# arkworks-rs/pcd

Hardware: AMD Instinct MI355X
Metric: msm_mscalar_mul_per_s (higher is better)
Workload: dtype u32 (11 x 28-bit unsaturated Montgomery limbs, v_mad_u64_u32 with 64-bit column accumulators); 1 GPU; MNT4-298 G1 variable-base MSM, n=1048576 pairs per GPU (2^20 per GPU), proving-key bases and scalars resident in HBM, scalar distribution uniform; curve=MNT4-298, group=G1, log_n=20, window_bits=20, windows=15

## Files before the change

### pcd_amd/csrc/capi_msm.hip

```cpp
#include <mutex>

#include "capi_internal.h"

using namespace pcd;

namespace {
__global__ void __launch_bounds__(256) zero_flagged_kernel(uint32_t* __restrict__ pts, const uint8_t* __restrict__ flags, size_t n_words,
                                                            uint32_t words_per_point) {
  const size_t i = (size_t)blockIdx.x * blockDim.x + threadIdx.x;
  if (i < n_words && flags[i / words_per_point]) pts[i] = 0;
}

int lane_reserve_of(const pcdhip_ctx* ctx) {
  int r = ctx->lane_reserve;
  if (r < 0) { const char* e = getenv("PCDHIP_LANE_RESERVE"); r = e ? atoi(e) : 8; }
  return r < 0 ? 0 : r;
}
hipStream_t masked_lane_of(int device, int cus, int reserve, hipError_t* err) {
  static std::mutex mu;
  static std::map<std::pair<int, int>, hipStream_t> pool;
  std::lock_guard<std::mutex> lock(mu);
  auto it = pool.find({device, reserve});
  if (it != pool.end()) { *err = hipSuccess; return it->second; }
  std::vector<uint32_t> mask((cus + 31) / 32, 0u);
  for (int i = 0; i < cus - reserve; i++) mask[i / 32] |= 1u << (i % 32);
  hipStream_t s = nullptr;
  *err = hipExtStreamCreateWithCUMask(&s, (uint32_t)mask.size(), mask.data());
  if (*err == hipSuccess) pool[{device, reserve}] = s;
  return s;
}
int make_side_streams(pcdhip_ctx* ctx) {
  int least = 0, greatest = 0;
  TRY(hipDeviceGetStreamPriorityRange(&least, &greatest));
  const bool lane_mode = ctx->g16_schedule == 2;
  int cus = 0;
  if (hipDeviceGetAttribute(&cus, hipDeviceAttributeMultiprocessorCount, ctx->device) != hipSuccess || cus <= 0) cus = 256;
  const int normal = (least + greatest) / 2;
  for (int k = 0; k < 6; k++) {
    int prio = lane_mode ? (k < 2 ? greatest : k < 4 ? normal : least) : (k < 2 ? greatest : k == 2 ? normal : least);
    static const char* side_prio = getenv("PCDHIP_SIDE_PRIO");
    if (side_prio && !strcmp(side_prio, "low")) prio = least;
    if (side_prio && !strcmp(side_prio, "mid")) prio = k < 3 ? normal : least;
    TRY(hipStreamCreateWithPriority(&ctx->g16_streams[k], hipStreamNonBlocking, prio));
    TRY(hipEventCreate(&ctx->g16_begin[k]));
    TRY(hipEventCreate(&ctx->g16_end[k]));
  }
  if (lane_mode) {
    int reserve = lane_reserve_of(ctx);
    if (reserve >= cus) reserve = 0;
    if (reserve > 0) {
      hipError_t e = hipSuccess;
      ctx->lane.stream = masked_lane_of(ctx->device, cus, reserve, &e);
      TRY(e);
    } else {
      TRY(hipStreamCreateWithPriority(&ctx->lane_stream, hipStreamNonBlocking, least));
      ctx->lane.stream = ctx->lane_stream;
    }
    ctx->lane.cus = cus - reserve;
  }
  TRY(hipEventCreateWithFlags(&ctx->g16_ready, hipEventDisableTiming));
  return PCDHIP_OK;
}
}

namespace pcd {
hipError_t zero_flagged(hipStream_t st, uint32_t* pts_dev, uint8_t* flags_dev, const uint8_t* flags_host, size_t n, size_t point_bytes) {
  if (!flags_host || !n) return hipSuccess;
  hipError_t e = hipMemcpyAsync(flags_dev, flags_host, n, hipMemcpyHostToDevice, st);
  if (e != hipSuccess) return e;
  const size_t nw = n * (point_bytes / 4);
  hipLaunchKernelGGL(zero_flagged_kernel, dim3((unsigned)((nw + 255) / 256)), dim3(256), 0, st, pts_dev, flags_dev, nw, (uint32_t)(point_bytes / 4));
  return hipGetLastError();
}

void shard_range(size_t n, size_t g, size_t parts, size_t* lo, size_t* hi) {
  const size_t base = n / parts, rem = n % parts;
  *lo = g * base + std::min(g, rem);
  *hi = *lo + base + (g < rem ? 1 : 0);
}
int bases_upload_single(pcdhip_ctx* ctx, int curve_id, int group_id, const uint64_t* xy, const uint8_t* inf, size_t n, pcdhip_bases** out) {
  BIND();
  const GroupEntry& ge = group_entry(curve_id, group_id);
  const size_t abi_b = (size_t)ge.point_abi_words * 4, int_b = (size_t)ge.base_stride_words * 4;
  pcdhip_bases* b = new (std::nothrow) pcdhip_bases();
  if (!b) return PCDHIP_E_OOM;
  b->curve_id = curve_id; b->group_id = group_id; b->n = n; b->dptr = nullptr; b->c = 0; b->groups = 1;
  if (ctx->precompute != 0 && n >= 64) {
    const bool full = ctx->precompute < 0;
    const int c = ctx->msm_c ? ctx->msm_c : std::max(6, msm_pick_window(n, ge.scalar_bits, full ? 1 : 0) + ctx->msm_c_bias);
    const int W = msm_num_windows(ge.scalar_bits, c);
    b->c = c;
    b->groups = full ? W : std::min(W, ctx->precompute);
  }
  hipError_t e = hipErrorOutOfMemory;
  while (true) {
    const size_t want = std::max<size_t>(n, 1) * int_b * b->groups;
    e = (ctx->precompute_budget && want > ctx->precompute_budget && b->groups > 1) ? hipErrorOutOfMemory : hipMalloc(&b->dptr, want);
    if (e == hipSuccess || b->groups == 1) break;
    (void)hipGetLastError();
    b->groups = (b->groups + 1) / 2;
  }
  if (e != hipSuccess) { (void)hipGetLastError(); delete b; return fail(ctx, e); }
  if (b->groups == 1) b->c = 0;
  e = ctx->aux_ws.ensure(AUX_MISC, std::max<size_t>(n, 1) * (abi_b + 1) + 64);
  char* stage = (char*)ctx->aux_ws.buf[AUX_MISC];
  if (e == hipSuccess) e = hipMemcpyAsync(stage, xy, n * abi_b, hipMemcpyHostToDevice, ctx->stream);
  if (e == hipSuccess) e = zero_flagged(ctx->stream, (uint32_t*)stage, (uint8_t*)stage + n * abi_b, inf, n, abi_b);
  if (e == hipSuccess) e = ge.points_in(ctx->stream, (const uint32_t*)stage, (uint32_t)n, b->dptr);
  if (e == hipSuccess && b->groups > 1) {
    const int W = msm_num_windows(ge.scalar_bits, b->c);
    const int Wg = (W + b->groups - 1) / b->groups;
    e = ge.precompute(ctx->stream, b->dptr, (uint32_t)n, b->groups, b->c * Wg);
  }
  if (e == hipSuccess && inf) {
    std::vector<uint32_t> bits((n + 31) / 32 + 1, 0u);
    bool any = false;
    for (size_t i = 0; i < n; i++) if (inf[i]) { bits[i >> 5] |= 1u << (i & 31); any = true; }
    if (any) {
      e = hipMalloc((void**)&b->inf_bits, bits.size() * 4);
      if (e == hipSuccess) e = hipMemcpyAsync(b->inf_bits, bits.data(), bits.size() * 4, hipMemcpyHostToDevice, ctx->stream);
      if (e == hipSuccess) e = hipStreamSynchronize(ctx->stream);
    }
  }
  if (e == hipSuccess) e = hipStreamSynchronize(ctx->stream);
  if (e != hipSuccess) { (void)hipFree(b->dptr); (void)hipFree(b->inf_bits); delete b; return fail(ctx, e); }
  *out = b;
  return PCDHIP_OK;
}

int msm_common(pcdhip_ctx* ctx, const pcdhip_bases* bases, size_t offset, const uint32_t* scalars_dev, size_t n,
               uint64_t* out_xyz, bool out_on_device) {
  const GroupEntry& ge = group_entry(bases->curve_id, bases->group_id);
  const size_t jac_b = (size_t)ge.point_words / 2 * 3 * 4, jac_abi_b = (size_t)ge.point_abi_words / 2 * 3 * 4;
  TRY(ctx->msm_ws.ensure(WS_OUT, jac_b + jac_abi_b + 64));
  uint32_t* out_dev = (uint32_t*)ctx->msm_ws.buf[WS_OUT];
  uint32_t* out_abi = out_dev + jac_b / 4;
  TRY(ge.msm(ctx->msm_ws, ctx->stream, bases->view(offset), scalars_dev, (uint32_t)n, out_dev, ctx->msm_c, ctx->msm_chunk,
             ctx->msm_sort, ctx->msm_profile ? &ctx->msm_tm : nullptr, nullptr, MSM_SHARE_NONE));
  if (out_on_device) { TRY(ge.jac_out(ctx->stream, out_dev, 1, (uint32_t*)out_xyz)); return PCDHIP_OK; }
  TRY(ge.jac_out(ctx->stream, out_dev, 1, out_abi));
  TRY(hipMemcpyAsync(out_xyz, out_abi, jac_abi_b, hipMemcpyDeviceToHost, ctx->stream));
  uint32_t too_wide = 0;
  if (ctx->msm_ws.last_err_dev) TRY(hipMemcpyAsync(&too_wide, ctx->msm_ws.last_err_dev, 4, hipMemcpyDeviceToHost, ctx->stream));
  TRY(hipStreamSynchronize(ctx->stream));
  return too_wide ? PCDHIP_E_ARG : PCDHIP_OK;
}

int ensure_side_streams(pcdhip_ctx* ctx) {
// ... 152 lines not shown
  uint32_t* d = (uint32_t*)ctx->aux_ws.buf[AUX_MISC];
  uint32_t* scratch = d + (n + 1) * jb / 4;
  const uint32_t* in = (const uint32_t*)xyz;
  if (!in_on_device) {
    TRY(hipMemcpyAsync(d + jb / 4, xyz, n * jb, hipMemcpyHostToDevice, ctx->stream));
    in = d + jb / 4;
  }
  TRY(ge.points_sum(ctx->stream, in, (uint32_t)n, scratch, d));
  TRY(hipMemcpyAsync(out_xyz, d, jb, hipMemcpyDeviceToHost, ctx->stream));
  TRY(hipStreamSynchronize(ctx->stream));
  return PCDHIP_OK;
}
}

extern "C" {

int pcdhip_bases_upload(pcdhip_ctx* ctx, int curve_id, int group_id, const uint64_t* xy, const uint8_t* inf, size_t n,
                        pcdhip_bases** out) {
  if (!ctx || !out || !valid_curve(curve_id) || !valid_group(group_id) || (!xy && n) || n >= (1ull << 31)) return PCDHIP_E_ARG;
  if (ctx->peers.size() <= 1) return bases_upload_single(ctx, curve_id, group_id, xy, inf, n, out);
  *out = nullptr;
  return guarded([&]() -> int {
    pcdhip_bases* b = new pcdhip_bases();
    b->curve_id = curve_id; b->group_id = group_id; b->n = n; b->dptr = nullptr; b->c = 0; b->groups = 1;
    const size_t G = ctx->peers.size(), pl = (size_t)pcdhip_point_limbs(curve_id, group_id);
    b->shard_lo.resize(G + 1);
    for (size_t g = 0; g < G; g++) {
      size_t lo, hi;
      shard_range(n, g, G, &lo, &hi);
      b->shard_lo[g] = lo; b->shard_lo[g + 1] = hi;
      pcdhip_ctx* C = ctx->peers[g];
      C->precompute = ctx->precompute; C->precompute_budget = ctx->precompute_budget; C->msm_c = ctx->msm_c;
      pcdhip_bases* sh = nullptr;
      int rc = bases_upload_single(C, curve_id, group_id, xy + lo * pl, inf ? inf + lo : nullptr, hi - lo, &sh);
      if (rc) { pcdhip_bases_free(ctx, b); return rc; }
      b->shards.push_back(sh);
    }
    *out = b;
    return PCDHIP_OK;
  });
}
int pcdhip_set_precompute(pcdhip_ctx* ctx, int mode) {
  if (!ctx || mode < -1 || mode == 1) return PCDHIP_E_ARG;
  ctx->precompute = mode;
  return PCDHIP_OK;
}
int pcdhip_set_precompute_budget(pcdhip_ctx* ctx, size_t bytes_per_vector) {
  if (!ctx) return PCDHIP_E_ARG;
  ctx->precompute_budget = bytes_per_vector;
  return PCDHIP_OK;
}
int pcdhip_get_precompute_budget(pcdhip_ctx* ctx, size_t* bytes_per_vector) {
  if (!ctx || !bytes_per_vector) return PCDHIP_E_ARG;
  *bytes_per_vector = ctx->precompute_budget;
  return PCDHIP_OK;
}
void pcdhip_bases_free(pcdhip_ctx* ctx, pcdhip_bases* bases) {
  if (!bases) return;
  for (size_t g = 0; g < bases->shards.size(); g++)
    pcdhip_bases_free(ctx && g < ctx->peers.size() ? ctx->peers[g] : ctx, bases->shards[g]);
  bases->shards.clear();
  if (ctx) (void)hipSetDevice(ctx->device);
  (void)hipFree(bases->dptr);
  (void)hipFree(bases->inf_bits);
  delete bases;
}
int pcdhip_bases_info(const pcdhip_bases* bases, size_t n, int* window_bits, int* windows, int* copies) {
  if (!bases || !window_bits || !windows || !copies) return PCDHIP_E_ARG;
  if (!bases->shards.empty()) return pcdhip_bases_info(bases->shards[0], 0, window_bits, windows, copies);
  const GroupEntry& ge = group_entry(bases->curve_id, bases->group_id);
  const int c = bases->groups > 1 ? bases->c : msm_pick_window(n ? n : bases->n, ge.scalar_bits, 0);
  *window_bits = c;
  *windows = msm_num_windows(ge.scalar_bits, c);
  *copies = bases->groups;
  return PCDHIP_OK;
}
int pcdhip_msm_config(pcdhip_ctx* ctx, int window_bits, int chunk) {
  if (!ctx || window_bits < 0 || window_bits > 24 || chunk < 0) return PCDHIP_E_ARG;
  ctx->msm_c = window_bits;
  ctx->msm_chunk = (uint32_t)chunk;
  return PCDHIP_OK;
}
int pcdhip_msm_set_sort(pcdhip_ctx* ctx, int mode) {
  if (!ctx || mode < 0 || mode > 2) return PCDHIP_E_ARG;
  ctx->msm_sort = (ctx->msm_sort & ~15) | mode;
  return PCDHIP_OK;
}
int pcdhip_msm_set_accumulate(pcdhip_ctx* ctx, int mode, int chunk, int min_pairs) {
  if (!ctx || mode < 0 || mode > 2 || chunk < 0 || chunk > 1024 || (chunk && chunk < 2) || min_pairs < 0 || min_pairs > 255) return PCDHIP_E_ARG;
  ctx->msm_sort = (ctx->msm_sort & 15) | (mode << 4) | (chunk << 8) | (min_pairs << 20);
  return PCDHIP_OK;
}
int pcdhip_msm_profile(pcdhip_ctx* ctx, int on) {
  if (!ctx) return PCDHIP_E_ARG;
  ctx->msm_profile = on != 0;
  return PCDHIP_OK;
}
int pcdhip_msm_last_plan(pcdhip_ctx* ctx, uint32_t out[2]) {
  if (!ctx || !out) return PCDHIP_E_ARG;
  out[0] = ctx->msm_tm.entries; out[1] = ctx->msm_tm.chunk;
  return PCDHIP_OK;
}
int pcdhip_msm_last_timings(pcdhip_ctx* ctx, float out_ms[8]) {
  if (!ctx || !out_ms) return PCDHIP_E_ARG;
  const MsmTimings& t = ctx->msm_tm;
  float v[8] = {t.digits, t.scan, t.scatter, t.accumulate, t.fixup, t.tail, t.horner, t.total};
  memcpy(out_ms, v, sizeof v);
  return PCDHIP_OK;
}

int pcdhip_msm_ticket_status(pcdhip_ctx* ctx, int slot) {
  if (!ctx || slot < 0 || slot >= pcdhip_ctx::PIPE_SLOTS || ctx->pipe_busy[slot] || !ctx->pipe_partial[slot]) return PCDHIP_E_ARG;
  BIND();
  TRY(hipEventSynchronize(ctx->pipe_done[slot]));
  ctx->pipe_partial[slot] = false;
  return (uint32_t)ctx->pipe_host[(size_t)slot * pcdhip_ctx::PIPE_HOST_WORDS + pcdhip_ctx::PIPE_HOST_WORDS - 1] ? PCDHIP_E_PREV_TICKET : PCDHIP_OK;
}
int pcdhip_msm_submit(pcdhip_ctx* ctx, const pcdhip_bases* bases, size_t offset, const pcdhip_buf* scalars, size_t scalar_offset, size_t n,
                      int* ticket) {
  const int rc = msm_submit_common(ctx, bases, offset, scalars, scalar_offset, n, nullptr, 0, ticket);
  return rc == PCDHIP_E_PREV_TICKET ? PCDHIP_OK : rc;
}
int pcdhip_msm_submit_partial(pcdhip_ctx* ctx, const pcdhip_bases* bases, size_t offset, const pcdhip_buf* scalars, size_t scalar_offset, size_t n,
                              uint64_t* out_xyz_device_slots, size_t slot_stride_bytes, int* ticket) {
  if (!out_xyz_device_slots || (slot_stride_bytes & 7)) return PCDHIP_E_ARG;
  return msm_submit_common(ctx, bases, offset, scalars, scalar_offset, n, out_xyz_device_slots, slot_stride_bytes, ticket);
}
int pcdhip_msm_ticket_wait(pcdhip_ctx* ctx, int ticket, void* other_stream) {
  if (!ctx || ticket < 0 || ticket >= pcdhip_ctx::PIPE_SLOTS || !ctx->pipe_busy[ticket]) return PCDHIP_E_ARG;
  BIND();
  TRY(hipStreamWaitEvent((hipStream_t)other_stream, ctx->pipe_done[ticket], 0));
  ctx->pipe_busy[ticket] = false;
  ctx->pipe_partial[ticket] = true;
  return PCDHIP_OK;
}
int pcdhip_msm_collect(pcdhip_ctx* ctx, int ticket, uint64_t* out_xyz) {
  if (!ctx || ticket < 0 || ticket >= pcdhip_ctx::PIPE_SLOTS || !ctx->pipe_busy[ticket] || !out_xyz) return PCDHIP_E_ARG;
  BIND();
  ctx->pipe_busy[ticket] = false;
  TRY(hipEventSynchronize(ctx->pipe_done[ticket]));
  const uint64_t* host = ctx->pipe_host + (size_t)ticket * pcdhip_ctx::PIPE_HOST_WORDS;
  memcpy(out_xyz, host, ctx->pipe_out_bytes[ticket]);
  return (uint32_t)host[pcdhip_ctx::PIPE_HOST_WORDS - 1] ? PCDHIP_E_ARG : PCDHIP_OK;
}

int pcdhip_msm_dev(pcdhip_ctx* ctx, const pcdhip_bases* bases, size_t offset, const pcdhip_buf* scalars, size_t scalar_offset,
                   size_t n, uint64_t* out_xyz) {
  if (!ctx || !bases || !scalars || !out_xyz) return PCDHIP_E_ARG;
  if (!bases->shards.empty()) return PCDHIP_E_ARG;
  if (offset + n > bases->n || scalar_offset + n > scalars->n || n >= (1ull << 31)) return PCDHIP_E_ARG;
  if (scalars->field_id != kCurveFr[bases->curve_id]) return PCDHIP_E_ARG;
  BIND();
  const size_t sw = (size_t)kFieldLimbs[scalars->field_id] * 2;
  return msm_common(ctx, bases, offset, scalars->dptr + scalar_offset * sw, n, out_xyz);
}

int pcdhip_msm_dev_partial(pcdhip_ctx* ctx, const pcdhip_bases* bases, size_t offset, const pcdhip_buf* scalars, size_t scalar_offset,
                           size_t n, uint64_t* out_xyz_device) {
  if (!ctx || !bases || !scalars || !out_xyz_device || !bases->shards.empty()) return PCDHIP_E_ARG;
  if (offset + n > bases->n || scalar_offset + n > scalars->n || n >= (1ull << 31)) return PCDHIP_E_ARG;
  if (scalars->field_id != kCurveFr[bases->curve_id]) return PCDHIP_E_ARG;
  BIND();
  const size_t sw = (size_t)kFieldLimbs[scalars->field_id] * 2;
  return msm_common(ctx, bases, offset, scalars->dptr + scalar_offset * sw, n, out_xyz_device, true);
}

int pcdhip_msm(pcdhip_ctx* ctx, const pcdhip_bases* bases, size_t offset, const uint64_t* scalars, size_t n, uint64_t* out_xyz) {
// ... 42 lines not shown
```

### pcd_amd/csrc/msm.hip.h

```cpp
#pragma once
#include <cstdlib>
#include <math.h>

#include <algorithm>
#include <type_traits>
#include <vector>

#include "ec.hip.h"

namespace pcd {

template <int K>
struct EventSet {
  hipEvent_t e[K] = {};
  bool live = false;
  hipError_t create() {
    for (int i = 0; i < K; i++) { hipError_t r = hipEventCreate(&e[i]); if (r != hipSuccess) return r; }
    live = true;
    return hipSuccess;
  }
  hipEvent_t operator[](int i) const { return e[i]; }
  ~EventSet() { for (int i = 0; i < K; i++) if (e[i]) (void)hipEventDestroy(e[i]); }
};

struct MsmPlan {
  uint32_t n = 0;
  int c = 0;
  int W = 0;
  uint32_t nkeys = 0;
  uint32_t chunk = 0;
};

PCD_HD constexpr int msm_num_windows(int scalar_bits, int c) { return (scalar_bits + c) / c; }

inline int msm_pick_window(size_t n, int scalar_bits, int full_precompute) {
  double best = 1e300;
  int bc = 8;
  for (int c = 6; c <= 22; c++) {
    int W = msm_num_windows(scalar_bits, c);
    int Wg = full_precompute ? 1 : W;
    double cost = (double)W * (double)n * 11.0 + (double)Wg * (double)(1u << c) * 16.0 * 1.3;
    int top = scalar_bits + 1 - (W - 1) * c;
    cost += (double)n / (double)(1u << (top > 20 ? 20 : top)) * 1400.0;
    if (cost < best) { best = cost; bc = c; }
  }
  return bc;
}

constexpr uint32_t MSM_NEG = 0x80000000u;
PCD_DEV uint32_t msm_signed(uint32_t raw, int c, uint32_t& carry, uint32_t& neg) {
  uint32_t d = raw + carry;
  const bool n = d > (1u << (c - 1));
  carry = n ? 1u : 0u;
  neg = n ? MSM_NEG : 0u;
  return n ? (1u << c) - d : d;
}
template <int NS>
PCD_DEV bool msm_scalar_too_wide(const uint32_t* s, int bits) {
  uint32_t o = 0;
#pragma unroll
  for (int k = 0; k < NS; k++) {
    if (32 * k >= bits) o |= s[k];
    else if (32 * (k + 1) > bits) o |= s[k] >> (bits - 32 * k);
  }
  return o != 0;
}
PCD_DEV bool msm_base_is_inf(const uint32_t* __restrict__ inf_bits, uint32_t idx) { return inf_bits && ((inf_bits[idx >> 5] >> (idx & 31u)) & 1u); }
template <int NS>
PCD_DEV uint32_t msm_digit(const uint32_t* s, int w, int c) {
  int bit = w * c;
  int word = bit >> 5, off = bit & 31;
  uint64_t x = s[word];
  if (word + 1 < NS) x |= (uint64_t)s[word + 1] << 32;
  return (uint32_t)(x >> off) & ((1u << c) - 1u);
}

enum { MODE_HIST = 0, MODE_SCATTER = 1, MODE_BIN = 2 };
template <int NS, int MODE>
__global__ void __launch_bounds__(256) msm_digits_kernel(const uint32_t* __restrict__ scalars, uint32_t n, int c, int W, int Wg,
                                                         uint32_t n_total, uint32_t base_offset, uint32_t nkeys,
                                                         uint32_t* __restrict__ cnt, const uint32_t* __restrict__ off,
                                                         uint32_t* __restrict__ sorted_idx, uint32_t* __restrict__ slots, uint32_t cap,
                                                         uint32_t* __restrict__ ones_idx, uint32_t* __restrict__ flag, int skip_ones,
                                                         int scalar_bits, uint32_t* __restrict__ err, const uint32_t* __restrict__ inf_bits) {
  if (MODE == MODE_SCATTER && flag && *flag == 0) return;
  uint32_t i = blockIdx.x * blockDim.x + threadIdx.x;
  bool live = i < n && !msm_base_is_inf(inf_bits, base_offset + i);
// ... 52 lines not shown
constexpr uint32_t MSM_MAX_BINS = 8192;

template <int NS, bool WRITE>
__global__ void __launch_bounds__(256) msm_coarse_kernel(const uint32_t* __restrict__ scalars, uint32_t n, int c, int W, int Wg,
                                                         uint32_t n_total, uint32_t base_offset, uint32_t nbins,
                                                         uint32_t* __restrict__ gbin ,
                                                         uint64_t* __restrict__ entries, uint32_t* __restrict__ ones_count,
                                                         uint32_t* __restrict__ ones_idx, int scalar_bits, uint32_t* __restrict__ err,
                                                         const uint32_t* __restrict__ inf_bits) {
  extern __shared__ uint32_t lbin[];
  __shared__ uint32_t s_ones[WRITE ? 1 : MSM_TILE];
  __shared__ uint32_t s_nones, s_ones_base;
  for (uint32_t b = threadIdx.x; b < nbins; b += blockDim.x) lbin[b] = 0;
  if (threadIdx.x == 0) s_nones = 0;
  __syncthreads();
  const uint32_t tile0 = blockIdx.x * MSM_TILE;
  for (uint32_t k = threadIdx.x; k < MSM_TILE; k += blockDim.x) {
    uint32_t i = tile0 + k;
    bool live = i < n && !msm_base_is_inf(inf_bits, base_offset + i);
    uint32_t s[NS];
    bool is_one = false;
    if (live || (i < n && !WRITE)) {
      uint32_t hi = 0;
#pragma unroll
      for (int q = 0; q < NS; q++) { s[q] = scalars[(size_t)i * NS + q]; if (q) hi |= s[q]; }
      is_one = live && (hi == 0 && s[0] == 1);
      if (!WRITE && msm_scalar_too_wide<NS>(s, scalar_bits)) *err = 1u;
    }
    if (!WRITE) {
      unsigned long long m = __ballot(live && is_one);
      if (m) {
        int lane = threadIdx.x & 63;
        int leader = __ffsll((long long)m) - 1;
        uint32_t base = 0;
        if (lane == leader) base = atomicAdd(&s_nones, (uint32_t)__popcll(m));
        base = __shfl(base, leader, 64);
        if (live && is_one) s_ones[base + (uint32_t)__popcll(m & ((1ull << lane) - 1ull))] = base_offset + i;
      }
    }
    if (!live || is_one) continue;
    int j = 0;
    uint32_t carry = 0, neg;
    for (int w = 0; w < W; w++) {
      uint32_t d = msm_signed(msm_digit<NS>(s, w, c), c, carry, neg);
      if (d != 0) atomicAdd(&lbin[((((uint32_t)j << c) | d)) >> MSM_BIN_SHIFT], 1u);
      if (++j == Wg) j = 0;
    }
  }
  __syncthreads();
  for (uint32_t b = threadIdx.x; b < nbins; b += blockDim.x) {
    uint32_t cnt = lbin[b];
    if (cnt) {
      uint32_t base = atomicAdd(&gbin[b], cnt);
      if (WRITE) lbin[b] = base;
    }
  }
  if (!WRITE) {
    if (threadIdx.x == 0) s_ones_base = s_nones ? atomicAdd(ones_count, s_nones) : 0u;
    __syncthreads();
    for (uint32_t k = threadIdx.x; k < s_nones; k += blockDim.x) ones_idx[s_ones_base + k] = s_ones[k];
    return;
  }
  __syncthreads();
  for (uint32_t k = threadIdx.x; k < MSM_TILE; k += blockDim.x) {
    uint32_t i = tile0 + k;
    if (i >= n || msm_base_is_inf(inf_bits, base_offset + i)) continue;
    uint32_t s[NS];
    uint32_t hi = 0;
#pragma unroll
    for (int q = 0; q < NS; q++) { s[q] = scalars[(size_t)i * NS + q]; if (q) hi |= s[q]; }
    if (hi == 0 && s[0] <= 1) continue;
    int g = 0, j = 0;
    uint32_t carry = 0, neg;
    for (int w = 0; w < W; w++) {
      uint32_t d = msm_signed(msm_digit<NS>(s, w, c), c, carry, neg);
      if (d != 0) {
        uint32_t key = ((uint32_t)j << c) | d;
        uint32_t pos = atomicAdd(&lbin[key >> MSM_BIN_SHIFT], 1u);
        entries[pos] = ((uint64_t)key << 32) | (uint64_t)(((uint32_t)g * n_total + base_offset + i) | neg);
      }
      if (++j == Wg) { j = 0; g++; }
    }
  }
}

static __global__ void __launch_bounds__(1024) msm_bin_scan_kernel(const uint32_t* __restrict__ bin_cnt, uint32_t nbins,
                                                                   uint32_t* __restrict__ bin_base, uint32_t* __restrict__ cursor,
                                                                   const uint32_t* __restrict__ ones_count, uint32_t* __restrict__ off,
                                                                   uint32_t nkeys) {
  __shared__ uint32_t part[1024];
  const uint32_t per = (nbins + 1023) / 1024;
  const uint32_t lo = threadIdx.x * per, hi = min(nbins, lo + per);
  uint32_t acc = 0;
  for (uint32_t b = lo; b < hi; b++) acc += bin_cnt[b];
  part[threadIdx.x] = acc;
  __syncthreads();
  for (int s = 1; s < 1024; s <<= 1) {
    uint32_t t = ((int)threadIdx.x >= s) ? part[threadIdx.x - s] : 0;
    __syncthreads();
    part[threadIdx.x] += t;
    __syncthreads();
  }
  uint32_t run = part[threadIdx.x] - acc;
  for (uint32_t b = lo; b < hi; b++) { bin_base[b] = run; cursor[b] = run; run += bin_cnt[b]; }
  if (threadIdx.x == 1023) {
    uint32_t M = part[1023];
    bin_base[nbins] = M;
    off[nkeys] = M;
    off[nkeys + 1] = M + *ones_count;
  }
}

static __global__ void __launch_bounds__(256) msm_bin_sort_kernel(const uint64_t* __restrict__ entries, const uint32_t* __restrict__ bin_base,
                                                                  uint32_t* __restrict__ sorted_idx, uint32_t* __restrict__ off) {
  constexpr uint32_t KB = 1u << MSM_BIN_SHIFT;
  __shared__ uint32_t hist[KB];
  __shared__ uint32_t wsum[4];
  const uint32_t b = blockIdx.x, lo = bin_base[b], hi = bin_base[b + 1];
  for (uint32_t k = threadIdx.x; k < KB; k += blockDim.x) hist[k] = 0;
  __syncthreads();
  for (uint32_t p0 = lo + threadIdx.x; p0 < hi; p0 += MSM_SORT_UNROLL * blockDim.x) {
    uint32_t kk[MSM_SORT_UNROLL];
#pragma unroll
    for (int u = 0; u < MSM_SORT_UNROLL; u++) { uint32_t p = p0 + u * blockDim.x; kk[u] = p < hi ? (uint32_t)(entries[p] >> 32) & (KB - 1) : KB; }
#pragma unroll
    for (int u = 0; u < MSM_SORT_UNROLL; u++) if (kk[u] < KB) atomicAdd(&hist[kk[u]], 1u);
  }
  __syncthreads();
  const uint32_t t = threadIdx.x, lane = t & 63, wv = t >> 6;
  uint32_t c0 = hist[2 * t], c1 = hist[2 * t + 1];
  uint32_t incl = c0 + c1;
  for (int d = 1; d < 64; d <<= 1) { uint32_t o = __shfl_up(incl, d, 64); if ((int)lane >= d) incl += o; }
  if (lane == 63) wsum[wv] = incl;
  __syncthreads();
  uint32_t before = 0;
  for (uint32_t q = 0; q < wv; q++) before += wsum[q];
  uint32_t ex = lo + before + incl - (c0 + c1);
  hist[2 * t] = ex;
  hist[2 * t + 1] = ex + c0;
  off[(size_t)b * KB + 2 * t] = ex;
  off[(size_t)b * KB + 2 * t + 1] = ex + c0;
  __syncthreads();
  for (uint32_t p0 = lo + threadIdx.x; p0 < hi; p0 += MSM_SORT_UNROLL * blockDim.x) {
    uint64_t e[MSM_SORT_UNROLL];
    uint32_t pos[MSM_SORT_UNROLL];
#pragma unroll
    for (int u = 0; u < MSM_SORT_UNROLL; u++) { uint32_t p = p0 + u * blockDim.x; e[u] = p < hi ? entries[p] : ~0ull; }
#pragma unroll
    for (int u = 0; u < MSM_SORT_UNROLL; u++) if (e[u] != ~0ull) pos[u] = atomicAdd(&hist[(uint32_t)(e[u] >> 32) & (KB - 1)], 1u);
#pragma unroll
    for (int u = 0; u < MSM_SORT_UNROLL; u++) if (e[u] != ~0ull) sorted_idx[pos[u]] = (uint32_t)e[u];
  }
}

static __global__ void __launch_bounds__(1024) scan_block_sums(const uint32_t* __restrict__ in, uint32_t n, uint32_t per_block,
                                                         uint32_t* __restrict__ block_sums) {
  __shared__ uint32_t sh[1024];
  uint32_t b = blockIdx.x, lo = b * per_block, hi = min(n, lo + per_block);
  uint32_t acc = 0;
  for (uint32_t i = lo + threadIdx.x; i < hi; i += blockDim.x) acc += in[i];
  sh[threadIdx.x] = acc;
  __syncthreads();
  for (int s = 512; s > 0; s >>= 1) { if ((int)threadIdx.x < s) sh[threadIdx.x] += sh[threadIdx.x + s]; __syncthreads(); }
  if (threadIdx.x == 0) block_sums[b] = sh[0];
}
static __global__ void __launch_bounds__(1024) scan_apply(const uint32_t* __restrict__ in, uint32_t n, uint32_t per_block,
// ... 1055 lines not shown
  const bool single_pass = sort_mode == 1;
  const uint32_t* bases_dev = bv.dptr;
  typedef typename G::F F;
  constexpr int NS = G::FR::N32;
  constexpr int PW = Jac<F>::WORDS;
  constexpr size_t PB = (size_t)PW * 4;
  if (n == 0) { ws.last_err_dev = nullptr; Jac<F> inf = Jac<F>::infinity(); return hipMemcpyAsync(out_dev, &inf, PB, hipMemcpyHostToDevice, st); }
  MsmPlan pl;
  pl.n = n;
  pl.c = bv.groups > 1 ? bv.c : (c_override ? c_override : msm_pick_window(n, G::FR::BITS, 0));
  pl.W = msm_num_windows(G::FR::BITS, pl.c);
  const int Wg = (pl.W + bv.groups - 1) / bv.groups;
  pl.nkeys = (uint32_t)Wg << pl.c;
  const uint64_t maxM = (uint64_t)n * pl.W;
  pl.chunk = chunk_override ? chunk_override : 40;
  int& cus = ws.cus;
  if (!cus) {
    int dev = 0;
    if (hipGetDevice(&dev) != hipSuccess || hipDeviceGetAttribute(&cus, hipDeviceAttributeMultiprocessorCount, dev) != hipSuccess || cus <= 0) cus = 256;
  }
  bool use_tree = false;
  uint32_t tree_cap = 0;
  const uint32_t* tree_chunk_dev = nullptr;
  if constexpr (MsmTreeCapable<G>::value) {
    use_tree = acc_mode == 2 && (uint64_t)bv.n_total * bv.groups < MSM_SCR;
    if (use_tree) {
      tree_cap = tree_chunk ? tree_chunk : MSM_TREE_CHUNK_MAX;
      pl.chunk = tree_cap;
    }
  }
  const MsmLane* lane = ws.lane;
  const int plan_cus = lane && lane->cus > 0 ? lane->cus : cus;
  uint32_t acc_lanes = 0, chunk_lo = 0;
  static const uint32_t chunk_hi_env = getenv("PCDHIP_CHUNK_HI") ? (uint32_t)atoi(getenv("PCDHIP_CHUNK_HI")) : 0u;
  const uint32_t chunk_hi = chunk_hi_env >= 16 && chunk_hi_env <= MSM_CHUNK_MAX ? chunk_hi_env : MSM_CHUNK_HI;
  if (!chunk_override && !use_tree) {
    acc_lanes = (uint32_t)plan_cus * 4 * MsmAccWaves<G>::value * (64 / AccOf<G>::LANES);
    chunk_lo = (uint32_t)std::min<uint64_t>(40, std::max<uint64_t>(16, (maxM + 4ull * acc_lanes - 1) / (4ull * acc_lanes)));
    pl.chunk = chunk_lo;
  }
  const uint64_t plan_word = acc_lanes && acc_lanes < (1u << 20) ? msm_plan_word(acc_lanes, chunk_lo, chunk_hi) : 0u;
  if (acc_lanes && !plan_word) pl.chunk = 40;
  if (maxM >= 0xFFFFFFF0ull || (uint64_t)bv.n_total * bv.groups >= 0x7FFFFFF0ull) return hipErrorInvalidValue;

  EventSet<9> ev;
  if (tm) PCD_HIP_TRY(ev.create());
  auto mark = [&](int i) -> hipError_t { return tm ? hipEventRecord(ev[i], st) : hipSuccess; };

  const uint32_t tkeys = pl.nkeys + 1, ones_key = pl.nkeys;
  const bool consume = share && share_role == MSM_SHARE_CONSUME && share->valid && share->n == n && share->n_total == bv.n_total &&
                       share->offset == bv.offset && share->tkeys == tkeys && share->c == pl.c && share->W == pl.W &&
                       share->groups == bv.groups && share->scalars == scalars_dev &&
                       (share->inf_bits == nullptr || share->inf_bits == bv.inf_bits);
  PCD_HIP_TRY(ws.ensure(WS_CNT, (size_t)tkeys * 4 + 16));
  PCD_HIP_TRY(ws.ensure(WS_OFF, ((size_t)tkeys + 1) * 4));
  const uint32_t scan_per_block = 16384;
  const uint32_t scan_blocks = (tkeys + scan_per_block - 1) / scan_per_block;
  PCD_HIP_TRY(ws.ensure(WS_BSUM, (size_t)scan_blocks * 4));
  PCD_HIP_TRY(ws.ensure(WS_SORTED, (size_t)maxM * 4));
  PCD_HIP_TRY(ws.ensure(WS_BUCKETS, (size_t)tkeys * PB));
  PCD_HIP_TRY(ws.ensure(WS_OUT, PB + 64));
  PCD_HIP_TRY(ws.ensure(WS_ONES, (size_t)n * 4 + 32));
  uint32_t* cnt = (uint32_t*)ws.buf[WS_CNT];
  uint32_t* off = (uint32_t*)ws.buf[WS_OFF];
  uint32_t* bsum = (uint32_t*)ws.buf[WS_BSUM];
  uint32_t* sorted = (uint32_t*)ws.buf[WS_SORTED];
  uint32_t* buckets = (uint32_t*)ws.buf[WS_BUCKETS];
  uint32_t* ones_idx = (uint32_t*)ws.buf[WS_ONES];
  uint32_t* flag = ones_idx + n;
  uint32_t* err = flag + 1;
  uint32_t* big_count = flag + 2;
  auto zero_start = [&](uint32_t n_cnt) {
    hipLaunchKernelGGL(msm_zero_kernel, dim3(std::max<uint32_t>(1u, (n_cnt + 255) / 256)), dim3(256), 0, st, cnt, n_cnt, flag);
  };
  ws.last_err_dev = consume ? nullptr : err;
  constexpr int SBITS = G::FR::BITS;
  const int wins = (pl.W + Wg - 1) / Wg;
  const int top_bits = G::FR::BITS + 1 - (pl.W - 1) * pl.c;
  double mu = (double)n * wins / (double)(1u << (pl.c - 1)) + (top_bits < pl.c ? (double)n / (double)(1u << top_bits) : 0.0);
  uint32_t cap = (uint32_t)(mu + 6.0 * sqrt(mu) + 8.0);
  cap = (cap + 7u) & ~7u;
  const bool use_slots = single_pass && (double)pl.nkeys * cap * 4.0 <= 1.5e9;
  const uint32_t nbins = pl.nkeys >> MSM_BIN_SHIFT;
  const bool use_partition = sort_mode == 0 && pl.c >= MSM_BIN_SHIFT && nbins >= 1 && nbins <= MSM_MAX_BINS && n >= 4096;
  uint32_t* slots = nullptr;
  if (use_slots) { PCD_HIP_TRY(ws.ensure(WS_SLOTS, (size_t)pl.nkeys * cap * 4)); slots = (uint32_t*)ws.buf[WS_SLOTS]; }

  PCD_HIP_TRY(mark(0));
  dim3 gd((n + 255) / 256), bd(256);
  MsmEntrySource src;
  if (consume) {
    PCD_HIP_TRY(hipStreamWaitEvent(st, share->ready, 0));
    zero_start(0);
    src = share->src;
    off = const_cast<uint32_t*>(share->off);
    PCD_HIP_TRY(mark(1)); PCD_HIP_TRY(mark(2)); PCD_HIP_TRY(mark(3));
  } else if (use_slots) {
    zero_start(tkeys);
    hipLaunchKernelGGL((msm_digits_kernel<NS, MODE_BIN>), gd, bd, 0, st, scalars_dev, n, pl.c, pl.W, Wg, bv.n_total, bv.offset, pl.nkeys, cnt,
                       (const uint32_t*)nullptr, (uint32_t*)nullptr, slots, cap, ones_idx, flag, 0, SBITS, err, bv.inf_bits);
    PCD_HIP_TRY(mark(1));
    hipLaunchKernelGGL(scan_block_sums, dim3(scan_blocks), dim3(1024), 0, st, cnt, tkeys, scan_per_block, bsum);
    hipLaunchKernelGGL(scan_apply, dim3(scan_blocks), dim3(1024), 0, st, cnt, tkeys, scan_per_block, bsum, scan_blocks, off);
    PCD_HIP_TRY(mark(2));
    PCD_HIP_TRY(ws.ensure(WS_CUR, (size_t)tkeys * 4));
    uint32_t* cur = (uint32_t*)ws.buf[WS_CUR];
    PCD_HIP_TRY(hipMemsetAsync(cur, 0, (size_t)tkeys * 4, st));
    hipLaunchKernelGGL((msm_digits_kernel<NS, MODE_SCATTER>), gd, bd, 0, st, scalars_dev, n, pl.c, pl.W, Wg, bv.n_total, bv.offset, pl.nkeys, cur,
                       off, sorted, (uint32_t*)nullptr, 0u, (uint32_t*)nullptr, flag, 1, SBITS, err, bv.inf_bits);
    PCD_HIP_TRY(mark(3));
    src = {sorted, slots, ones_idx, flag, cap, ones_key};
  } else if (use_partition) {
    zero_start(nbins + 1);
    const uint32_t tiles = (n + MSM_TILE - 1) / MSM_TILE;
    PCD_HIP_TRY(ws.ensure(WS_ENTRIES, (size_t)maxM * 8));
    PCD_HIP_TRY(ws.ensure(WS_CUR, ((size_t)2 * nbins + 8) * 4));
    uint64_t* entries = (uint64_t*)ws.buf[WS_ENTRIES];
    uint32_t* bin_base = (uint32_t*)ws.buf[WS_CUR];
    uint32_t* cursor = bin_base + nbins + 2;
    uint32_t* ones_count = flag;
    hipLaunchKernelGGL((msm_coarse_kernel<NS, false>), dim3(tiles), dim3(256), (size_t)nbins * 4, st, scalars_dev, n, pl.c, pl.W, Wg, bv.n_total,
                       bv.offset, nbins, cnt, (uint64_t*)nullptr, ones_count, ones_idx, SBITS, err, bv.inf_bits);
    PCD_HIP_TRY(mark(1));
    hipLaunchKernelGGL(msm_bin_scan_kernel, dim3(1), dim3(1024), 0, st, cnt, nbins, bin_base, cursor, ones_count, off, pl.nkeys);
    PCD_HIP_TRY(mark(2));
    hipLaunchKernelGGL((msm_coarse_kernel<NS, true>), dim3(tiles), dim3(256), (size_t)nbins * 4, st, scalars_dev, n, pl.c, pl.W, Wg, bv.n_total,
                       bv.offset, nbins, cursor, entries, ones_count, ones_idx, SBITS, err, bv.inf_bits);
    hipLaunchKernelGGL(msm_bin_sort_kernel, dim3(nbins), dim3(256), 0, st, entries, bin_base, sorted, off);
    PCD_HIP_TRY(mark(3));
    src = {sorted, nullptr, ones_idx, nullptr, 0u, ones_key};
  } else {
    zero_start(tkeys);
    hipLaunchKernelGGL((msm_digits_kernel<NS, MODE_HIST>), gd, bd, 0, st, scalars_dev, n, pl.c, pl.W, Wg, bv.n_total, bv.offset, pl.nkeys, cnt,
                       (const uint32_t*)nullptr, (uint32_t*)nullptr, (uint32_t*)nullptr, 0u, (uint32_t*)nullptr, (uint32_t*)nullptr, 0, SBITS, err, bv.inf_bits);
    PCD_HIP_TRY(mark(1));
    hipLaunchKernelGGL(scan_block_sums, dim3(scan_blocks), dim3(1024), 0, st, cnt, tkeys, scan_per_block, bsum);
    hipLaunchKernelGGL(scan_apply, dim3(scan_blocks), dim3(1024), 0, st, cnt, tkeys, scan_per_block, bsum, scan_blocks, off);
    PCD_HIP_TRY(mark(2));
    PCD_HIP_TRY(hipMemsetAsync(cnt, 0, (size_t)tkeys * 4, st));
    hipLaunchKernelGGL((msm_digits_kernel<NS, MODE_SCATTER>), gd, bd, 0, st, scalars_dev, n, pl.c, pl.W, Wg, bv.n_total, bv.offset, pl.nkeys, cnt,
                       off, sorted, (uint32_t*)nullptr, 0u, (uint32_t*)nullptr, (uint32_t*)nullptr, 0, SBITS, err, bv.inf_bits);
    PCD_HIP_TRY(mark(3));
    src = {sorted, nullptr, nullptr, nullptr, 0u, ones_key};
  }
  if (share && share_role == MSM_SHARE_PRODUCE) {
    share->valid = true;
    share->n = n; share->n_total = bv.n_total; share->offset = bv.offset; share->tkeys = tkeys;
    share->c = pl.c; share->W = pl.W; share->groups = bv.groups; share->scalars = scalars_dev; share->inf_bits = bv.inf_bits;
    share->src = src; share->off = off;
    PCD_HIP_TRY(hipEventRecord(share->ready, st));
  }
  uint32_t nchunks = (uint32_t)((maxM + pl.chunk - 1) / pl.chunk);
  uint32_t tree_grid = 0;
  if (use_tree) {
    tree_grid = std::min<uint32_t>(tree_chunk ? (nchunks + 63) / 64 : (uint32_t)((maxM / 32 + 63) / 64), (uint32_t)plan_cus * 4);
    if (!tree_chunk) nchunks = tree_grid * 64 * (uint32_t)((maxM + (uint64_t)tree_grid * 64 * tree_cap - 1) / ((uint64_t)tree_grid * 64 * tree_cap));
  }
  typedef MsmStored<typename SplitOf<G>::type> Stored;
  constexpr size_t RB = (size_t)Stored::WORDS * 4;
  PCD_HIP_TRY(ws.ensure(WS_PFIRST, (size_t)nchunks * RB));
  PCD_HIP_TRY(ws.ensure(WS_PLAST, (size_t)nchunks * RB));
  uint32_t* acc_buckets = buckets;
  if (Stored::SEPARATE) { PCD_HIP_TRY(ws.ensure(WS_ACCB, (size_t)tkeys * RB)); acc_buckets = (uint32_t*)ws.buf[WS_ACCB]; }
  const uint32_t big_limit = 8, seg_len = 128;
  const uint32_t big_cap = nchunks / big_limit + 2;
  const uint32_t seg_cap = nchunks / seg_len + big_cap + 2;
  PCD_HIP_TRY(ws.ensure(WS_BIG, (size_t)(3 * big_cap + 3 * seg_cap + 8) * 4));
  PCD_HIP_TRY(ws.ensure(WS_BIGPART, (size_t)seg_cap * PB));
  uint32_t* pfirst = (uint32_t*)ws.buf[WS_PFIRST];
  uint32_t* plast = (uint32_t*)ws.buf[WS_PLAST];
  uint32_t* big = (uint32_t*)ws.buf[WS_BIG];
  uint32_t* seg_list = big + 3 * big_cap;
  uint32_t* big_partial = (uint32_t*)ws.buf[WS_BIGPART];
  PCD_HIP_TRY(mark(8));
  hipStream_t own = st;
  if (lane) {
    if (!ws.lane_in) PCD_HIP_TRY(hipEventCreateWithFlags(&ws.lane_in, hipEventDisableTiming));
    if (!ws.lane_out) PCD_HIP_TRY(hipEventCreateWithFlags(&ws.lane_out, hipEventDisableTiming));
    PCD_HIP_TRY(hipEventRecord(ws.lane_in, own));
    PCD_HIP_TRY(hipStreamWaitEvent(lane->stream, ws.lane_in, 0));
    st = lane->stream;
  }
  {
    constexpr uint32_t per_wave = 64 / AccOf<G>::LANES;
    const dim3 acc_grid((nchunks + per_wave - 1) / per_wave);
    bool launched = false;
    if constexpr (MsmTreeCapable<G>::value) {
      if (use_tree) {
        constexpr int FW = AccOf<G>::type::F::WORDS;
        const uint32_t grid = tree_grid;
        MsmTreeBufs tb;
        tb.cap = tree_cap;
        tb.phases = 3;
        uint32_t* chunk_word = big_count + 2;
        hipLaunchKernelGGL(msm_tree_plan_kernel, dim3(1), dim3(1), 0, st, off, tkeys, grid * 64, tree_cap, tree_chunk, chunk_word);
        tree_chunk_dev = chunk_word;
        PCD_HIP_TRY(ws.ensure(WS_TLIST, MsmTreeBufs::list_words(tb.cap) * 4 * grid));
        PCD_HIP_TRY(ws.ensure(WS_TPAIR, MsmTreeBufs::pair_words(tb.cap) * 4 * grid));
        PCD_HIP_TRY(ws.ensure(WS_TPREFIX, MsmTreeBufs::prefix_words(tb.cap, FW) * 4 * grid));
        PCD_HIP_TRY(ws.ensure(WS_TPTS, MsmTreeBufs::pts_words(tb.cap, FW) * 4 * grid));
        tb.list = (uint32_t*)ws.buf[WS_TLIST]; tb.pairs = (uint32_t*)ws.buf[WS_TPAIR];
        tb.prefix = (uint32_t*)ws.buf[WS_TPREFIX]; tb.pts = (uint32_t*)ws.buf[WS_TPTS];
        hipLaunchKernelGGL((msm_pair_tree_kernel<G>), dim3(grid), dim3(64), 0, st, bases_dev, src, off, tkeys, chunk_word, tb,
                           tree_min_pairs ? tree_min_pairs : MSM_TREE_MIN_PAIRS, acc_buckets, pfirst, plast);
        launched = true;
      }
    }
    if (!launched) {
      if (src.slots) hipLaunchKernelGGL((msm_accumulate_kernel<G, false>), acc_grid, dim3(64), 0, st, bases_dev, src, off, tkeys, pl.chunk, acc_buckets, pfirst, plast, plan_word);
      hipLaunchKernelGGL((msm_accumulate_kernel<G, true>), acc_grid, dim3(64), 0, st, bases_dev, src, off, tkeys, pl.chunk, acc_buckets, pfirst, plast, plan_word);
// ... 94 lines not shown
```

Baseline: 398.7 Mscalar-mul/s.

## Stage coarse-partition scatter in LDS to write contiguous per-bin runs

Adds a staged coarse scatter kernel for the partition sort path. Each block histograms its tile's digits in LDS and reserves one global range per bin with a single atomic. It then packs entries into an LDS buffer ordered by bin and writes them out as contiguous runs, replacing per-entry global atomics and scattered 64-bit writes. The trade-off is large dynamic LDS use (up to 152 KB), which lowers occupancy, plus a binary search per entry. An env knob can cap or disable the tile, and sort mode 3 keeps the old path.

```diff
diff --git a/pcd_amd/csrc/capi_msm.hip b/pcd_amd/csrc/capi_msm.hip
--- a/pcd_amd/csrc/capi_msm.hip
+++ b/pcd_amd/csrc/capi_msm.hip
@@ -64,6 +64,16 @@
 }
 
 namespace pcd {
+int msm_coarse_tile_knob() {
+  static const int knob = [] {
+    const char* e = getenv("PCDHIP_COARSE_TILE");
+    if (!e || *e < '0' || *e > '9') return -1;
+    const int v = atoi(e);
+    return v == 0 || (v >= (int)MSM_STAGE_TILE_MIN && v <= (int)MSM_STAGE_TILE_MAX) ? v : -1;
+  }();
+  return knob;
+}
+
 hipError_t zero_flagged(hipStream_t st, uint32_t* pts_dev, uint8_t* flags_dev, const uint8_t* flags_host, size_t n, size_t point_bytes) {
   if (!flags_host || !n) return hipSuccess;
   hipError_t e = hipMemcpyAsync(flags_dev, flags_host, n, hipMemcpyHostToDevice, st);
@@ -382,7 +392,7 @@
   return PCDHIP_OK;
 }
 int pcdhip_msm_set_sort(pcdhip_ctx* ctx, int mode) {
-  if (!ctx || mode < 0 || mode > 2) return PCDHIP_E_ARG;
+  if (!ctx || mode < 0 || mode > 3) return PCDHIP_E_ARG;
   ctx->msm_sort = (ctx->msm_sort & ~15) | mode;
   return PCDHIP_OK;
 }
diff --git a/pcd_amd/csrc/msm.hip.h b/pcd_amd/csrc/msm.hip.h
--- a/pcd_amd/csrc/msm.hip.h
+++ b/pcd_amd/csrc/msm.hip.h
@@ -3,6 +3,7 @@
 #include <math.h>
 
 #include <algorithm>
+#include <atomic>
 #include <type_traits>
 #include <vector>
 
@@ -221,6 +222,134 @@
       if (++j == Wg) { j = 0; g++; }
     }
   }
+}
+
+constexpr int MSM_STAGE_G_BITS = 6, MSM_STAGE_IDX_BITS = 11;
+constexpr uint32_t MSM_STAGE_TILE_MAX = 1u << MSM_STAGE_IDX_BITS, MSM_STAGE_TILE_MIN = 256;
+constexpr int MSM_STAGE_W_MAX = 1 << MSM_STAGE_G_BITS;
+constexpr int MSM_STAGE_SIGN_AT = MSM_BIN_SHIFT, MSM_STAGE_G_AT = MSM_BIN_SHIFT + 1, MSM_STAGE_IDX_AT = MSM_STAGE_G_AT + MSM_STAGE_G_BITS;
+static_assert(MSM_STAGE_IDX_AT + MSM_STAGE_IDX_BITS <= 32, "staged word: low key bits, sign, group and tile index in 32 bits");
+constexpr size_t MSM_STAGE_LDS_BUDGET = 152u * 1024u;
+constexpr uint32_t MSM_STAGE_MIN_RUN = 8;
+PCD_HD constexpr size_t msm_stage_lds_bytes(uint32_t tile, int W, uint32_t nbins) { return 4 * ((size_t)tile * (size_t)W + 3 * (size_t)nbins + 4); }
+PCD_HD constexpr uint32_t msm_stage_tile(int W, uint32_t nbins) {
+  if (W < 1 || W > MSM_STAGE_W_MAX || nbins < 1) return 0;
+  for (uint32_t t = MSM_STAGE_TILE_MAX; t >= MSM_STAGE_TILE_MIN; t >>= 1)
+    if (msm_stage_lds_bytes(t, W, nbins) <= MSM_STAGE_LDS_BUDGET) return (uint64_t)t * (uint32_t)W >= (uint64_t)MSM_STAGE_MIN_RUN * nbins ? t : 0;
+  return 0;
+}
+int msm_coarse_tile_knob();
+
+constexpr int msm_stage_block(int TILE) { return TILE < 1024 ? TILE : 1024; }
+template <int NS, int TILE>
+__global__ void __launch_bounds__(msm_stage_block(TILE)) msm_coarse_staged_kernel(const uint32_t* __restrict__ scalars, uint32_t n, int c, int W, int Wg,
+                                                                                  uint32_t n_total, uint32_t base_offset, uint32_t nbins,
+                                                                                  uint32_t* __restrict__ gbin ,
+                                                                                  uint64_t* __restrict__ entries, const uint32_t* __restrict__ inf_bits) {
+  constexpr int BLOCK = msm_stage_block(TILE), K = TILE / BLOCK, NW = BLOCK / 64;
+  static_assert(TILE >= (int)MSM_STAGE_TILE_MIN && TILE <= (int)MSM_STAGE_TILE_MAX && TILE % BLOCK == 0, "tile");
+  extern __shared__ uint32_t lds[];
+  uint32_t* cur = lds;
+  uint32_t* loff = cur + nbins;
+  uint32_t* rdelta = loff + nbins + 1;
+  uint32_t* buf = rdelta + nbins;
+  __shared__ uint32_t s_wsum[NW];
+  const uint32_t t = threadIdx.x, tile0 = blockIdx.x * TILE;
+  for (uint32_t b = t; b < nbins; b += BLOCK) cur[b] = 0;
+  uint32_t s[K][NS];
+  bool live[K];
+#pragma unroll
+  for (int kk = 0; kk < K; kk++) {
+    const uint32_t i = tile0 + t + kk * BLOCK;
+    live[kk] = i < n && !msm_base_is_inf(inf_bits, base_offset + i);
+    uint32_t hi = 0;
+#pragma unroll
+    for (int q = 0; q < NS; q++) { s[kk][q] = live[kk] ? scalars[(size_t)i * NS + q] : 0u; if (q) hi |= s[kk][q]; }
+    if (hi == 0 && s[kk][0] <= 1) live[kk] = false;
+  }
+  __syncthreads();
+#pragma unroll
+  for (int kk = 0; kk < K; kk++) {
+    if (!live[kk]) continue;
+    int j = 0;
+    uint32_t carry = 0, neg;
+    for (int w = 0; w < W; w++) {
+      uint32_t d = msm_signed(msm_digit<NS>(s[kk], w, c), c, carry, neg);
+      if (d != 0) atomicAdd(&cur[((((uint32_t)j << c) | d)) >> MSM_BIN_SHIFT], 1u);
+      if (++j == Wg) j = 0;
+    }
+  }
+  __syncthreads();
+  const uint32_t per = (nbins + BLOCK - 1) / BLOCK;
+  const uint32_t blo = min(nbins, t * per), bhi = min(nbins, blo + per);
+  uint32_t acc = 0;
+  for (uint32_t b = blo; b < bhi; b++) acc += cur[b];
+  const uint32_t lane = t & 63, wv = t >> 6;
+  uint32_t incl = acc;
+  for (int d = 1; d < 64; d <<= 1) { uint32_t o = __shfl_up(incl, d, 64); if ((int)lane >= d) incl += o; }
+  if (lane == 63) s_wsum[wv] = incl;
+  __syncthreads();
+  uint32_t run = incl - acc;
+  for (uint32_t q = 0; q < wv; q++) run += s_wsum[q];
+  for (uint32_t b = blo; b < bhi; b++) {
+    const uint32_t cnt = cur[b];
+    loff[b] = run;
+    cur[b] = run;
+    if (cnt) rdelta[b] = atomicAdd(&gbin[b], cnt) - run;
+    run += cnt;
+  }
+  if (t == BLOCK - 1) loff[nbins] = run;
+  __syncthreads();
+#pragma unroll
+  for (int kk = 0; kk < K; kk++) {
+    if (!live[kk]) continue;
+    int g = 0, j = 0;
+    uint32_t carry = 0, neg;
+    for (int w = 0; w < W; w++) {
+      uint32_t d = msm_signed(msm_digit<NS>(s[kk], w, c), c, carry, neg);
+      if (d != 0) {
+        const uint32_t key = ((uint32_t)j << c) | d;
+        const uint32_t q = atomicAdd(&cur[key >> MSM_BIN_SHIFT], 1u);
+        buf[q] = (key & ((1u << MSM_BIN_SHIFT) - 1u)) | (neg ? 1u << MSM_STAGE_SIGN_AT : 0u) | ((uint32_t)g << MSM_STAGE_G_AT) |
+                 ((t + kk * BLOCK) << MSM_STAGE_IDX_AT);
+      }
+      if (++j == Wg) { j = 0; g++; }
+    }
+  }
+  __syncthreads();
+  const uint32_t total = loff[nbins];
+  for (uint32_t q = t; q < total; q += BLOCK) {
+    const uint32_t word = buf[q];
+    uint32_t lo = 0, hi = nbins;
+    while (hi - lo > 1) {
+      const uint32_t mid = (lo + hi) >> 1;
+      if (loff[mid] <= q) lo = mid; else hi = mid;
+    }
+    const uint32_t key = (lo << MSM_BIN_SHIFT) | (word & ((1u << MSM_BIN_SHIFT) - 1u));
+    const uint32_t g = (word >> MSM_STAGE_G_AT) & ((1u << MSM_STAGE_G_BITS) - 1u);
+    const uint32_t neg = (word >> MSM_STAGE_SIGN_AT) & 1u ? MSM_NEG : 0u;
+    const uint32_t idx = (g * n_total + base_offset + tile0 + (word >> MSM_STAGE_IDX_AT)) | neg;
+    entries[rdelta[lo] + q] = ((uint64_t)key << 32) | (uint64_t)idx;
+  }
+}
+template <int NS, int TILE>
+hipError_t msm_coarse_staged_launch(hipStream_t st, uint32_t tiles, size_t lds, const uint32_t* scalars, uint32_t n, int c, int W, int Wg,
+                                    uint32_t n_total, uint32_t base_offset, uint32_t nbins, uint32_t* gbin, uint64_t* entries,
+                                    const uint32_t* inf_bits) {
+  static std::atomic<uint64_t> allowed{0};
+  int dev = 0;
+  hipError_t e = hipGetDevice(&dev);
+  if (e != hipSuccess) return e;
+  const uint64_t bit = 1ull << (dev & 63);
+  if (!(allowed.load(std::memory_order_relaxed) & bit)) {
+    e = hipFuncSetAttribute(reinterpret_cast<const void*>(&msm_coarse_staged_kernel<NS, TILE>), hipFuncAttributeMaxDynamicSharedMemorySize,
+                            (int)MSM_STAGE_LDS_BUDGET);
+    if (e != hipSuccess) return e;
+    allowed.fetch_or(bit, std::memory_order_relaxed);
+  }
+  hipLaunchKernelGGL((msm_coarse_staged_kernel<NS, TILE>), dim3(tiles), dim3(msm_stage_block(TILE)), lds, st, scalars, n, c, W, Wg, n_total,
+                     base_offset, nbins, gbin, entries, inf_bits);
+  return hipSuccess;
 }
 
 static __global__ void __launch_bounds__(1024) msm_bin_scan_kernel(const uint32_t* __restrict__ bin_cnt, uint32_t nbins,
@@ -1442,7 +1571,13 @@
   cap = (cap + 7u) & ~7u;
   const bool use_slots = single_pass && (double)pl.nkeys * cap * 4.0 <= 1.5e9;
   const uint32_t nbins = pl.nkeys >> MSM_BIN_SHIFT;
-  const bool use_partition = sort_mode == 0 && pl.c >= MSM_BIN_SHIFT && nbins >= 1 && nbins <= MSM_MAX_BINS && n >= 4096;
+  const bool use_partition = (sort_mode == 0 || sort_mode == 3) && pl.c >= MSM_BIN_SHIFT && nbins >= 1 && nbins <= MSM_MAX_BINS && n >= 4096;
+  uint32_t stage_tile = 0;
+  if (use_partition && sort_mode == 0) {
+    const int knob = msm_coarse_tile_knob();
+    stage_tile = knob == 0 ? 0u : msm_stage_tile(pl.W, nbins);
+    while (knob > 0 && stage_tile > (uint32_t)knob) stage_tile >>= 1;
+  }
   uint32_t* slots = nullptr;
   if (use_slots) { PCD_HIP_TRY(ws.ensure(WS_SLOTS, (size_t)pl.nkeys * cap * 4)); slots = (uint32_t*)ws.buf[WS_SLOTS]; }
 
@@ -1484,8 +1619,16 @@
     PCD_HIP_TRY(mark(1));
     hipLaunchKernelGGL(msm_bin_scan_kernel, dim3(1), dim3(1024), 0, st, cnt, nbins, bin_base, cursor, ones_count, off, pl.nkeys);
     PCD_HIP_TRY(mark(2));
-    hipLaunchKernelGGL((msm_coarse_kernel<NS, true>), dim3(tiles), dim3(256), (size_t)nbins * 4, st, scalars_dev, n, pl.c, pl.W, Wg, bv.n_total,
-                       bv.offset, nbins, cursor, entries, ones_count, ones_idx, SBITS, err, bv.inf_bits);
+    if (stage_tile) {
+      const uint32_t stiles = (n + stage_tile - 1) / stage_tile;
+      const size_t lds = msm_stage_lds_bytes(stage_tile, pl.W, nbins);
+#define PCD_STAGED(T) msm_coarse_staged_launch<NS, T>(st, stiles, lds, scalars_dev, n, pl.c, pl.W, Wg, bv.n_total, bv.offset, nbins, cursor, entries, bv.inf_bits)
+      PCD_HIP_TRY(stage_tile == 2048 ? PCD_STAGED(2048) : stage_tile == 1024 ? PCD_STAGED(1024) : stage_tile == 512 ? PCD_STAGED(512) : PCD_STAGED(256));
+#undef PCD_STAGED
+    } else {
+      hipLaunchKernelGGL((msm_coarse_kernel<NS, true>), dim3(tiles), dim3(256), (size_t)nbins * 4, st, scalars_dev, n, pl.c, pl.W, Wg, bv.n_total,
+                         bv.offset, nbins, cursor, entries, ones_count, ones_idx, SBITS, err, bv.inf_bits);
+    }
     hipLaunchKernelGGL(msm_bin_sort_kernel, dim3(nbins), dim3(256), 0, st, entries, bin_base, sorted, off);
     PCD_HIP_TRY(mark(3));
     src = {sorted, nullptr, ones_idx, nullptr, 0u, ones_key};
```

After: 405.6 Mscalar-mul/s, median of 6. 1.02x the previous value.
